# adfriend45/HYBRID9

Measured on AMD Instinct MI355X. Metric: grid-cell-steps/sec at 0.5° global (1/2/4/8 GPUs) + achieved HBM GB/s, higher is better.
Workload: dtype f32

## Files before the change

### hybrid9_amd/csrc/h9g_pair.h

```cpp
#pragma once
#include "h9g_step.h"
#if !defined(__HIPCC__) && !defined(__HIP__)
#define __device__
#define __forceinline__ inline
#endif

#ifndef H9G_EXACT_HOOK
#define H9G_EXACT_HOOK(k0, ns)
#endif
#if defined(H9G_COUNT_EXACT)
__device__ unsigned long long h9g_exact_count;
__device__ unsigned h9g_exact_wave[1 << 16];
#endif
namespace h9k {

enum : int {
  PF_TS = 0, PF_HKS, PF_BSW, PF_PSI,
  PF_NINVB,
  PF_ITS,
  PF_PTE,
  PF_C3,
  PF_ROOTR,
  PF_RPSI0, PF_RPSI1,
  PF_RTS0, PF_RTS1,
  PF_SVH2O, PF_SVSMP,
  PF_N
};
enum : int {
  PS_FMAX = 0, PS_MH3, PS_TSDZ1, PS_DAY,
  PS_LAI = PS_DAY + D_N,
  PS_LAIL, PS_PM, PS_PFM, PS_PLEN, PS_RDEPTH,
  PS_DR0,
  PS_DRS = PS_DR0 + 4 * DRP_N,
  PS_SVZWT = PS_DR0 + 2 * DR_N,
  PS_SVWA, PS_SVRNF, PS_SVERR, PS_SVNS,
  PS_N
};
enum : int { SV_ZWT = 0, SV_WA, SV_RNF, SV_ERR, SV_NS };
static_assert((PS_DAY + D_NUMC) % 2 == 0 && (PS_DAY + D_RAARAC) % 2 == 0 && (PS_DAY + D_DGRAC) % 2 == 0 &&
                  (PS_DAY + D_DRR) % 2 == 0 && (PS_DAY + D_RAC) % 2 == 0 && PS_DR0 % 2 == 0,
              "pair fields must start a row");

#ifndef H9G_FE_EQ
#define H9G_FE_EQ 1
#endif
#ifndef H9G_FE_HK
#define H9G_FE_HK 1
#endif
#ifndef H9G_FE2
#define H9G_FE2 1
#endif
#ifndef H9G_SPARE_FENCE
#define H9G_SPARE_FENCE 0
#endif
#ifndef H9G_INL_LAST
#define H9G_INL_LAST 1
#endif
#ifndef H9G_EB_FAST
#define H9G_EB_FAST 1
#endif
#ifndef H9G_HK_MDIV
#define H9G_HK_MDIV 1
#endif
#ifndef H9G_INL_MDIV
#define H9G_INL_MDIV 0
#endif
#ifndef H9G_WT_DEFER
#define H9G_WT_DEFER 1
#endif
#ifndef H9G_AQ_FREE
#define H9G_AQ_FREE 0
#endif
#ifndef H9G_SPARE_L10
#define H9G_SPARE_L10 0
#endif

#ifndef H9G_P1_TASKS
#define H9G_P1_TASKS 1
#endif

template <int K>
struct FV {
  float v[K];
};

H9K_HD float sel(int h, float a, float b) { return h ? b : a; }
H9K_HD double seld(int h, double a, double b) { return h ? b : a; }

H9K_HD float pair_swap(float v) {
#if defined(__HIP_DEVICE_COMPILE__)
  const int x = __builtin_bit_cast(int, v);
  return __builtin_bit_cast(float, __builtin_amdgcn_update_dpp(x, x, 0xB1, 0xF, 0xF, false));
#else
  return v;
#endif
}

template <int E>
H9K_HD float pair_bcast(float v) {
#if defined(__HIP_DEVICE_COMPILE__)
  const int x = __builtin_bit_cast(int, v);
  return __builtin_bit_cast(float, __builtin_amdgcn_mov_dpp(x, E ? 0xF5 : 0xA0, 0xF, 0xF, true));
#else
  return v;
#endif
}

H9K_HD float lane_get(float v, int src) {
#if defined(__HIP_DEVICE_COMPILE__)
  return __builtin_bit_cast(float, __builtin_amdgcn_ds_bpermute(src << 2, __builtin_bit_cast(int, v)));
#else
  (void)src;
  return v;
#endif
}
H9K_HD int lane_geti(int v, int src) {
#if defined(__HIP_DEVICE_COMPILE__)
  return __builtin_amdgcn_ds_bpermute(src << 2, v);
#else
  (void)src;
  return v;
#endif
}

H9K_HD float lane0_get(float v) {
#if defined(__HIP_DEVICE_COMPILE__)
  return __builtin_bit_cast(float, __builtin_amdgcn_readlane(__builtin_bit_cast(int, v), 0));
#else
  return v;
#endif
}
H9K_HD int lane0_geti(int v) {
#if defined(__HIP_DEVICE_COMPILE__)
  return __builtin_amdgcn_readlane(v, 0);
#else
  return v;
#endif
}
H9K_HD uint64_t lane_mask(bool p) {
#if defined(__HIP_DEVICE_COMPILE__)
  return __builtin_amdgcn_ballot_w64(p);
#else
  return p ? 1u : 0u;
#endif
}

H9K_HD double join_d(float lo, float hi) {
  return __builtin_bit_cast(double, (uint64_t)__builtin_bit_cast(uint32_t, hi) << 32 |
                                        __builtin_bit_cast(uint32_t, lo));
}
H9K_HD float lo_d(double v) { return __builtin_bit_cast(float, (uint32_t)__builtin_bit_cast(uint64_t, v)); }
H9K_HD float hi_d(double v) {
  return __builtin_bit_cast(float, (uint32_t)(__builtin_bit_cast(uint64_t, v) >> 32));
}

template <int L>
struct FlatStore {
  static constexpr bool kRecip = true, kRts = true, kDayRecip = true, kRtsHK = true, kSpare = false;
  static constexpr int FE_EQ = 1, FE_HK = 1;
  static constexpr int N = PF_N * L + PS_N;
  float *b;
// ... 595 lines not shown
          const float d = sp.own_sc(cs, PS_DAY + D_RAC, h);
          auto rr = [&]() __attribute__((always_inline)) { return sp.own_day_rp(cs, DRP_RA, h); };
          const float LEh = mdiv(sp.own_sc(cs, PS_DAY + D_DRR, h) + ddiv(DC(D_RHOCP) * VDD0f, d, rr),
                                 desatdT + gamma * (1.0f + ddiv(r, d, rr)));
          return FV<1>{{ddiv(LEh * 1.0E3f, DC(D_RL), [&]() { return cs.day_r(DR_RL); })}};
        },
        ft, fe);
#if defined(H9G_FORCE_RERUN)
    bad |= (__builtin_bit_cast(uint32_t, theta[1]) & 15u) == 0;
#endif
    if (!__builtin_expect(any_lane(bad), 0)) {
      rsc = rscf;
      tran = ft.v[0];
      evg = fe.v[0];
      eb_fast = true;
    }
  }
  if (!eb_fast) {
  H9G_BR(BR_EBX);
  if ((DC(D_OK) != zero) && (beta > zero))
    rsc = DC(D_X) / (DC(D_LAI2) * beta * DC(D_PW28));
  else
    rsc = 1.0E6f;
  rsc = MAXF(rsc, DC(D_RSCMIN));
  FV<2> ebc, ebs;
  sp.template pick<2>(
      [&](int h) __attribute__((always_inline)) -> FV<2> {
        const float r = sel(h, rsc, rss);
        const float q = divr<CS::kDayRecip>(m, r, sp.own_sc(cs, PS_DAY + D_RAARAC, h),
                                            [&]() { return sp.own_day_rp(cs, DRP_RAARA, h); });
        const float PM = sp.own_sc(cs, PS_DAY + D_NUMC, h) / (desatdT + gamma * (one + q));
        const float R = sp.own_sc(cs, PS_DAY + D_DGRAC, h) + gamma * r;
        return FV<2>{{PM, R}};
      },
      ebc, ebs);
  const float PMc = ebc.v[0], Rc = ebc.v[1], PMs = ebs.v[0], Rs = ebs.v[1];
  FV<1> ccf, csf;
  sp.template pick<1>(
      [&](int h) __attribute__((always_inline)) -> FV<1> {
        const float Rh = sel(h, Rc, Rs), Ro = sel(h, Rs, Rc);
        return FV<1>{{one / (one + Rh * Ra / (Ro * (Rh + Ra)))}};
      },
      ccf, csf);
  const float LE = ccf.v[0] * PMc + csf.v[0] * PMs;
  const float VDD0 = DC(D_VDD) + divr<CS::kDayRecip>(m, (DC(D_A1) - DC(D_DG) * LE) * DC(D_RAA), DC(D_RHOCP),
                                                     [&]() { return cs.day_r(DR_RHOCP); });
  FV<1> ftr, fev;
  sp.template pick<1>(
      [&](int h) __attribute__((always_inline)) -> FV<1> {
        const float r = sel(h, rsc, rss);
        const float d = sp.own_sc(cs, PS_DAY + D_RAC, h);
        auto rr = [&]() __attribute__((always_inline)) { return sp.own_day_rp(cs, DRP_RA, h); };
        const float LEh = (sp.own_sc(cs, PS_DAY + D_DRR, h) + divr<CS::kDayRecip>(m, DC(D_RHOCP) * VDD0, d, rr)) /
                          (desatdT + gamma * (1.0f + divr<CS::kDayRecip>(m, r, d, rr)));
        return FV<1>{{divr<CS::kDayRecip>(m, LEh * 1.0E3f, DC(D_RL), [&]() { return cs.day_r(DR_RL); })}};
      },
      ftr, fev);
  tran = ftr.v[0];
  evg = fev.v[0];
  }
  float em1 = m.div(g.dz(1) * (theta[1] - watmin), dt, g.rdt()) - tran * ROOT(1);
  em1 = MAXF(zero, em1);
  evg = MINF(em1, evg);
  pr.flux(evg, tran);
  const float qflx_evap = evg;
  float qflx_in_soil = (one - frac_h2osfc) * (qflx_top_soil - qflx_surf);
  qflx_in_soil = qflx_in_soil - (one - frac_h2osfc) * qflx_evap;
  const float qinmax = (one - fsat) * cs.sc(PS_MH3);
  const float qflx_infl_excess = MAXF(zero, qflx_in_soil - (one - frac_h2osfc) * qinmax);
  const float qflx_infl = qflx_in_soil - qflx_infl_excess;
  qflx_surf = qflx_surf + qflx_infl_excess;
  float zwtmm = 1000.0f * s.zwt;
  const int jwt = jwt_of<L>(s.zwt, zim);
  const bool aq = (jwt == L);
  cs.launder();
  pr.mark(1);

  float zq[L + 2];
  float hk[L + 1], dhkdw[L + 1], dsmpdw[L + 1];
  constexpr bool kTask = pair1_tasks<M, SP, CS>();
  FV<1> p0{{zero}}, p1{{zero}};
  FV<2> eA{{zero, zero}}, eS{{zero, zero}};
  bool picks = true, aq_task = false;
  {
    float *const outq[1] = {zq};
    float *const outk[4] = {hk, dhkdw, smp, dsmpdw};
    auto eq_exact = [&](int t, int h) __attribute__((always_inline)) -> FV<1> {
          H9G_BR(BR_EQX);
          const int i0 = 2 * t + 1;
          const int il = i0 + h;
          const float zlo = cs.zi(il - 1), zhi = cs.zi(il);
          const float ts = OWN(PF_TS), psi = OWN(PF_PSI);
          float vol_eq;
          if (zwtmm <= zlo) {
            vol_eq = ts;
          } else {
            const float expo = one + OWN(PF_NINVB);
            auto rp = [&]() __attribute__((always_inline)) {
              return join_d(OWN(PF_RPSI0), OWN(PF_RPSI1));
            };
            const bool inl = (zwtmm < zhi) && (zwtmm > zlo);
            const float n0 = ((-psi) + zwtmm - zlo), ni = (-psi + zwtmm - zhi);
            bool bq = false;
            float b0 = divr_d<CS::kRecip>(m, n0, -psi, rp, bq);
            float bi = divr_d<CS::kRecip>(m, ni, -psi, rp, bq);
            if (__builtin_expect(bq, 0)) {
              divr_fix<CS::kRecip>(m, b0, n0, -psi);
              divr_fix<CS::kRecip>(m, bi, ni, -psi);
            }
            bi = inl ? one : bi;
            bool s0, si;
            float temp0 = m.powf_d(b0, expo, s0);
            float tpi = m.powf_d(bi, expo, si);
            if (__builtin_expect(s0 | si, 0)) {
              m.powf_fix(temp0, b0, expo, s0);
              m.powf_fix(tpi, bi, expo, si);
            }
            if (inl) {
              const float tempi = one;
              const float voleq1 = OWN(PF_PTE) / (zwtmm - zlo) * (tempi - temp0);
              vol_eq = m.div(voleq1 * (zwtmm - zlo) + ts * (zhi - zwtmm), zhi - zlo, cs.rdz_t(il));
              vol_eq = MINF(ts, vol_eq);
              vol_eq = MAXF(vol_eq, zero);
            } else {
              const float tempi = tpi;
              vol_eq = OWN(PF_C3) * (tempi - temp0);
              vol_eq = MAXF(vol_eq, 0.0f);
              vol_eq = MINF(ts, vol_eq);
            }
          }
          const float qv = divr<CS::kRts>(m, vol_eq, ts, [&]() { return join_d(OWN(PF_RTS0), OWN(PF_RTS1)); });
          float z = psi * m.powf(MAXX(qv, 0.01f), -OWN(PF_BSW));
          return FV<1>{{MAXC(smpmin, z)}};
    };
    auto eq_body = [&](int il, auto O, float zw, bool &bad, bool inl_all) __attribute__((always_inline)) -> FV<1> {
          const float zlo = cs.zi(il - 1), zhi = cs.zi(il);
          const float ts = O(PF_TS), psi = O(PF_PSI);
          const bool sat = zw <= zlo;
          const bool inl = (zw < zhi) && (zw > zlo);
          const float expo = one + O(PF_NINVB);
          auto rp = [&]() __attribute__((always_inline)) { return join_d(O(PF_RPSI0), O(PF_RPSI1)); };
          const float n0 = ((-psi) + zw - zlo), ni = (-psi + zw - zhi);
          float b0 = divr_d<CS::kRecip>(m, n0, -psi, rp, bad);
          float bi = divr_d<CS::kRecip>(m, ni, -psi, rp, bad);
          b0 = sat ? one : b0;
          bi = (sat || inl) ? one : bi;
          bool s0, si;
          const float temp0 = m.powf_d(b0, expo, s0);
          const float tpi = m.powf_d(bi, expo, si);
          bad |= s0 | si;
          float vin = zero;
          if (inl_all || any_lane(inl)) {
          H9G_BR(BR_INL);
          const float d0 = zw - zlo;
#if H9G_INL_MDIV
          bool bq = false;
          const float q1 = mk_div(O(PF_PTE), d0, bq);
#else
          const float q1 = m.div_d(O(PF_PTE), d0, recip64(d0));
          const bool bq = m.div_bad(q1);
#endif
          const float voleq1 = q1 * (one - temp0);
          vin = m.div_d(voleq1 * (zw - zlo) + ts * (zhi - zw), zhi - zlo, cs.rdz_t(il));
          bad |= inl && (bq | m.div_bad(vin));
          vin = MINF(ts, vin);
          vin = MAXF(vin, zero);
// ... 7 lines not shown
          const float z = psi * m.powf_d(MAXX(qv, 0.01f), -O(PF_BSW), sz);
          bad |= sz;
          return FV<1>{{MAXC(smpmin, z)}};
    };
    auto eq_fast = [&](int t, int h, bool &bad) __attribute__((always_inline)) -> FV<1> {
          return eq_body(2 * t + 1 + h, [&](int p) __attribute__((always_inline)) { return OWN(p); }, zwtmm, bad,
                         false);
    };
    auto hk_exact = [&](int t, int h) __attribute__((always_inline)) -> FV<4> {
          H9G_BR(BR_HKX);
          const int i0 = 2 * t + 1;
          const int ip1 = (L < i0 + 2) ? L : i0 + 2;
          const float th = sel(h, theta[i0], theta[i0 + 1]);
          const float thp = sel(h, theta[i0 + 1], theta[ip1]);
          const float ts = OWN(PF_TS);
          const float tsp = sel(h, TS(i0 + 1), TS(ip1));
          float s1 = 0.5f * (th + thp) / (0.5f * (ts + tsp));
          s1 = MINC(one, s1);
          const float bsw = OWN(PF_BSW);
          float s_node = MAXX(divr<CS::kRtsHK>(m, th, ts, [&]() { return join_d(OWN(PF_RTS0), OWN(PF_RTS1)); }),
                              0.01f);
          s_node = MINC(one, s_node);
          const float ek = 2.0f * bsw + 2.0f, es = -bsw;
          bool sk, ss;
          float pk = m.powf_d(s1, ek, sk);
          float ps = m.powf_d(s_node, es, ss);
          if (__builtin_expect(sk | ss, 0)) {
            m.powf_fix(pk, s1, ek, sk);
            m.powf_fix(ps, s_node, es, ss);
          }
          const float s2 = OWN(PF_HKS) * pk;
          FV<4> r;
          r.v[0] = s1 * s2;
          r.v[1] = (2.0f * bsw + 3.0f) * s2 * OWN(PF_ITS);
          float sm = OWN(PF_PSI) * ps;
          sm = MAXC(smpmin, sm);
          r.v[2] = sm;
          r.v[3] = (-bsw) * sm / (s_node * ts);
          return r;
    };
    auto hk_body = [&](auto O, float th, float thp, float tsp, bool &bad) __attribute__((always_inline)) -> FV<4> {
          const float ts = O(PF_TS);
          const float sa = th + thp, sb = ts + tsp, its = O(PF_ITS);
          const float q0 = sa * its;
          float s1 = __builtin_fmaf(__builtin_fmaf(-sb, q0, sa), its, q0);
          const uint32_t ua = __builtin_bit_cast(uint32_t, sa) - 0x21800000u;
          const uint32_t ub = __builtin_bit_cast(uint32_t, sb) - 0x21800000u;
          bad |= (ua > ub ? ua : ub) >= 0x5d800000u - 0x21800000u;
          s1 = MINC(one, s1);
          const float bsw = O(PF_BSW);
          float s_node = MAXX(divr_d<CS::kRtsHK>(m, th, ts, [&]() { return join_d(O(PF_RTS0), O(PF_RTS1)); }, bad),
                              0.01f);
          s_node = MINC(one, s_node);
          const float ek = 2.0f * bsw + 2.0f, es = -bsw;
          bool sk, ss;
          const float pk = m.powf_d(s1, ek, sk);
          const float ps = m.powf_d(s_node, es, ss);
          bad |= sk | ss;
          const float s2 = O(PF_HKS) * pk;
          FV<4> r;
          r.v[0] = s1 * s2;
          r.v[1] = (2.0f * bsw + 3.0f) * s2 * O(PF_ITS);
          float sm = O(PF_PSI) * ps;
          sm = MAXC(smpmin, sm);
          r.v[2] = sm;
          if constexpr (H9G_HK_MDIV && L <= 8)
            r.v[3] = mk_div((-bsw) * sm, s_node * ts, bad);
          else
            r.v[3] = (-bsw) * sm / (s_node * ts);
          return r;
    };
    auto hk_fast = [&](int t, int h, bool &bad) __attribute__((always_inline)) -> FV<4> {
          const int i0 = 2 * t + 1;
          const int ip1 = (L < i0 + 2) ? L : i0 + 2;
          return hk_body([&](int p) __attribute__((always_inline)) { return OWN(p); }, sel(h, theta[i0], theta[i0 + 1]),
                         sel(h, theta[i0 + 1], theta[ip1]), sel(h, TS(i0 + 1), TS(ip1)), bad);
    };
    if constexpr (kTask) {
      constexpr int NA = 4 * L + 2;
      (void)outq;
      static_assert(NA <= 64 && CS::kRecip && CS::kRts && CS::kRtsHK, "a lane per task, every reciprocal stored");
      const bool st = sp.spare;
      const int hh = sp.h;
      int ln = sp.ln;
      opaque(ln);
      if (!st) {
#pragma unroll
        for (int t = 0; t < NT; t++) cs.wb[CS::TH0 + 2 * t + hh] = sel(hh, theta[2 * t + 1], theta[2 * t + 2]);
      }
      const float zw = lane0_get(zwtmm);
      const int jwu = lane0_geti(jwt);
      const bool aqu = jwu == L;
      const int jcu = aqu ? L : jwu + 1;
      const int ta = ln < NA ? ln : NA - 1;
      const bool lay_a = ta < 4 * L;
      const int ka = lay_a ? (ta & 3) : ta - 4 * L + 4;
      const int ia = lay_a ? (ta >> 2) + 1 : jcu;
      const int ipa = ia < L ? ia + 1 : L;
      const lds_float *oa = cs.wb + (ia - 1);
      const float th = oa[CS::TH0], thp = cs.wb[CS::TH0 + ipa - 1];
      const float ts_a = oa[PF_TS * L], psi_a = oa[PF_PSI * L], bsw_a = oa[PF_BSW * L];
      const float ninv_a = oa[PF_NINVB * L], its_a = oa[PF_ITS * L], hks_a = oa[PF_HKS * L];
      const float pte_a = oa[PF_PTE * L], c3_a = oa[PF_C3 * L];
      const float tsp_a = cs.wb[PF_TS * L + ipa - 1];
      const double rpsi_a = join_d(oa[PF_RPSI0 * L], oa[PF_RPSI1 * L]);
      const double rts_a = join_d(oa[PF_RTS0 * L], oa[PF_RTS1 * L]);
      const float zlo_a = cs.zi(ia - 1), zhi_a = cs.zi(ia);
      const bool sat_a = zw <= zlo_a, inl_a = (zw < zhi_a) && (zw > zlo_a);
      const float sa = th + thp, sb = ts_a + tsp_a;
      const float q0 = sa * its_a;
      float s1 = __builtin_fmaf(__builtin_fmaf(-sb, q0, sa), its_a, q0);
      const uint32_t ua = __builtin_bit_cast(uint32_t, sa) - 0x21800000u;
      const uint32_t ub = __builtin_bit_cast(uint32_t, sb) - 0x21800000u;
      const bool s1bad = (ua > ub ? ua : ub) >= 0x5d800000u - 0x21800000u;
      s1 = MINC(one, s1);
      const bool by_ts = ka == 2 || ka == 3 || (ka == 4 && !aqu);
      const float nz = (-psi_a + zw) - (ka == 0 ? zlo_a : zhi_a);
      const float num_a = by_ts ? th : (ka == 5 ? zw : nz);
      const float q_a = m.div_d(num_a, by_ts ? ts_a : -psi_a, by_ts ? rts_a : rpsi_a);
      float sn_a = MAXX(q_a, 0.01f);
      sn_a = MINC(one, sn_a);
      const bool one_a = (ka == 0 && sat_a) || (ka == 1 && (sat_a || inl_a));
      const float x_a = ka == 2 ? s1 : (by_ts ? sn_a : (ka == 5 ? one + q_a : (one_a ? one : q_a)));
      const float e_a = (ka <= 1 || (ka == 4 && aqu)) ? one + ninv_a
                        : ka == 2                     ? 2.0f * bsw_a + 2.0f
                        : ka == 3                     ? -bsw_a
                        : ka == 4                     ? 2.0f * bsw_a + 3.0f
                                                      : ninv_a;
      bool sw_a;
      const float w_a = m.powf_d(x_a, e_a, sw_a);
      bool f_a = m.div_bad(q_a) | sw_a | (ka == 2 && s1bad);
      const float s2 = hks_a * w_a;
      const float o_hk = x_a * s2;
      const float o_dhk = (2.0f * bsw_a + 3.0f) * s2 * its_a;
      float o_sm = psi_a * w_a;
      o_sm = MAXC(smpmin, o_sm);
      float o_ds;
      if constexpr (H9G_HK_MDIV && L <= 8) {
        bool b3 = false;
        o_ds = mk_div((-bsw_a) * o_sm, x_a * ts_a, b3);
        f_a |= ka == 3 && b3;
      } else {
        o_ds = (-bsw_a) * o_sm / (x_a * ts_a);
      }
      const float t0 = pair_bcast<0>(w_a);
      const bool inl1 = inl_a && ka == 1;
      float vin = zero;
      if (any_lane(inl1)) {
        H9G_BR(BR_INL);
        const float d0 = zw - zlo_a;
#if H9G_INL_MDIV
        bool bq = false;
        const float q1 = mk_div(pte_a, d0, bq);
#else
        const float q1 = m.div_d(pte_a, d0, recip64(d0));
        const bool bq = m.div_bad(q1);
#endif
        const float voleq1 = q1 * (one - t0);
        vin = m.div_d(voleq1 * (zw - zlo_a) + ts_a * (zhi_a - zw), zhi_a - zlo_a, cs.rdz_t(ia));
        f_a |= inl1 && (bq | m.div_bad(vin));
        vin = MINF(ts_a, vin);
        vin = MAXF(vin, zero);
      }
      float vbl = c3_a * (w_a - t0);
      vbl = MAXF(vbl, 0.0f);
      vbl = MINF(ts_a, vbl);
      const float vol_eq = sat_a ? ts_a : (inl_a ? vin : vbl);
      float ve = zero;
      if (aqu) {
        const float d0 = zw - g.zi(L);
        ve = pte_a / d0 * (1.0f - w_a);
        ve = MAXF(ve, 0.0f);
        ve = MINF(ts_a, ve);
      }
      const uint64_t fl_a = lane_mask(f_a);
      pr.mark(2);
      const float num_b = ka == 4 ? ve : (ka == 5 ? th : vol_eq);
      const float q_b = m.div_d(num_b, ts_a, rts_a);
      const float xm_b = MAXX(q_b, 0.01f);
      float sn_b = MAXX(0.5f * (one + q_b), 0.01f);
      sn_b = MINC(one, sn_b);
      const float x_b = ka >= 4 ? (aqu ? (ka == 4 ? xm_b : sn_b) : one) : xm_b;
      bool sw_b;
      const float w_b = m.powf_d(x_b, -bsw_a, sw_b);
      float o_z = psi_a * w_b;
      o_z = MAXC(smpmin, o_z);
      float o_dz = zero;
      if (aqu) o_dz = -bsw_a * o_z / (x_b * ts_a);
      const uint64_t fl_b = lane_mask((m.div_bad(q_b) | sw_b) && (ka == 1 || (ka >= 4 && aqu)));
      int vz = 0;
      opaque(vz);
#pragma unroll
      for (int i = 1; i <= L; i++) {
        const int lb = 4 * (i - 1);
        zq[i] = lane_get(o_z, vz + lb + 1);
        hk[i] = lane_get(o_hk, vz + lb + 2);
        dhkdw[i] = lane_get(o_dhk, vz + lb + 2);
        smp[i] = lane_get(o_sm, vz + lb + 3);
        dsmpdw[i] = lane_get(o_ds, vz + lb + 3);
      }
      p0.v[0] = lane_get(w_a, vz + 4 * L);
      p1.v[0] = lane_get(w_a, vz + 4 * L + 1);
      if (aqu) {
        eA.v[0] = lane_get(o_z, vz + 4 * L);
        eS.v[0] = lane_get(o_z, vz + 4 * L + 1);
        eS.v[1] = lane_get(o_dz, vz + 4 * L + 1);
      }
      if (st) return 0;
      constexpr uint64_t ALL_A = (1ull << (4 * L)) - 1;
      const bool bad_eq = (((fl_a & 0x3333333333333333ull) | (fl_b & 0x2222222222222222ull)) & ALL_A) != 0;
      const bool bad_hk = (fl_a & 0xCCCCCCCCCCCCCCCCull & ALL_A) != 0;
      if (__builtin_expect(bad_eq, 0)) {
#pragma unroll
        for (int t = 0; t < NT; t++) {
          const FV<1> r = eq_exact(t, hh);
          sp.xchg(r.v[0], zq[2 * t + 1], zq[2 * t + 2]);
        }
      }
      if (__builtin_expect(bad_hk, 0)) {
#pragma unroll
        for (int t = 0; t < NT; t++) {
          const FV<4> r = hk_exact(t, hh);
#pragma unroll
          for (int kk = 0; kk < 4; kk++) sp.xchg(r.v[kk], outk[kk][2 * t + 1], outk[kk][2 * t + 2]);
        }
      }
      aq_task = aqu;
      picks = ((fl_a >> (4 * L)) & 3) != 0 || (aqu && ((fl_b >> (4 * L)) & 3) != 0);
    } else if constexpr (SP::kSpare && CS::kSpare && !M::kExact) {
      constexpr int S = CS::LANES, H = 64 - S;
      constexpr int R = (NT * S + 63) / 64, U = NT - R, TOT = U * S;
      static_assert(U >= 1 && TOT <= R * H, "the helpers cover the first U slots in R rounds");
      const bool st = sp.spare;
      const int hh = sp.h;
      auto tau_q = [&](int q) __attribute__((always_inline)) {
        const int t = q * H + (st ? sp.ln - S : 0);
        return t < TOT ? t : TOT - 1;
      };
      auto src_u = [&](int u) __attribute__((always_inline)) { return S + (u * S + sp.ln) % H; };
      auto qo_u = [&](int u) __attribute__((always_inline)) { return (u * S + sp.ln) / H; };
      auto qlo = [](int u) constexpr { return (u * S) / H; };
      auto qhi = [](int u) constexpr { return ((u * S + S - 1) / H) < R - 1 ? (u * S + S - 1) / H : R - 1; };
      auto ulo = [](int q) constexpr { return (q * H) / S < U - 1 ? (q * H) / S : U - 1; };
      auto uhi = [](int q) constexpr { return (q * H + H - 1) / S < U - 1 ? (q * H + H - 1) / S : U - 1; };
      auto back = [&](const float (&v)[R], int u) __attribute__((always_inline)) {
        const int src = src_u(u), qo = qo_u(u);
        float x = lane_get(v[qlo(u)], src);
#pragma unroll
        for (int q = qlo(u) + 1; q <= qhi(u); q++) {
          const float g = lane_get(v[q], src);
          x = qo == q ? g : x;
        }
        return x;
      };
      auto flags_back = [&](int fl) __attribute__((always_inline)) {
        bool any = false;
#pragma unroll
        for (int u = 0; u < U; u++) any |= ((lane_geti(fl, src_u(u)) >> qo_u(u)) & 1) != 0;
        return any;
      };
      {
        float zwk[R];
#pragma unroll
        for (int q = 0; q < R; q++) zwk[q] = lane_get(zwtmm, tau_q(q) % S);
        FV<1> r[NT];
        float rv[R];
        int fl = 0;
#pragma unroll
        for (int q = 0; q < R; q++) {
          const int tau = tau_q(q), k = tau % S, u = tau / S;
          const int t = U + q;
          const lds_float *o = st ? cs.wb + k + u * S : cs.self + t * S;
          bool b = false;
          r[t] = eq_body(st ? 2 * u + 1 + (k & 1) : 2 * t + 1 + hh,
                         [&](int p) __attribute__((always_inline)) { return o[p * NT * S]; },
                         st ? zwk[q] : zwtmm, b, H9G_INL_LAST && U + q == NT - 1);
          rv[q] = r[t].v[0];
          fl |= (b ? 1 : 0) << q;
          if ((H9G_SPARE_FENCE >> q) & 1) sched_fence();
        }
#pragma unroll
        for (int u = 0; u < U; u++) r[u].v[0] = back(rv, u);
        const bool bad = !st & ((fl != 0) | flags_back(fl));
        if (__builtin_expect(bad, 0)) {
#pragma unroll
          for (int t = 0; t < NT; t++) r[t] = eq_exact(t, hh);
        }
#pragma unroll
        for (int t = 0; t < NT; t++) sp.xchg(r[t].v[0], zq[2 * t + 1], zq[2 * t + 2]);
      }
      pr.mark(2);
      {
        float thu[U], thpu[U];
#pragma unroll
        for (int u = 0; u < U; u++) {
          thu[u] = sel(hh, theta[2 * u + 1], theta[2 * u + 2]);
          thpu[u] = sel(hh, theta[2 * u + 2], theta[2 * u + 3]);
        }
        float thk[R], thpk[R];
#pragma unroll
        for (int q = 0; q < R; q++) {
          const int tau = tau_q(q), k = tau % S, u = tau / S;
          float a = lane_get(thu[ulo(q)], k), b = lane_get(thpu[ulo(q)], k);
#pragma unroll
          for (int w = ulo(q) + 1; w <= uhi(q); w++) {
            const float ga = lane_get(thu[w], k), gb = lane_get(thpu[w], k);
            a = u == w ? ga : a;
            b = u == w ? gb : b;
          }
          thk[q] = a;
          thpk[q] = b;
// ... 78 lines not shown
        return FV<1>{{w}};
      },
      p0, p1);
  const FV<1> pA = p0;
  if (any_aq) {
  H9G_BR(BR_ANYAQ);
  {
    const float d0 = aq ? (zwtmm - g.zi(L)) : one;
    float ve = LAYF(PF_PTE, L) / d0 * (1.0f - pA.v[0]);
    ve = MAXF(ve, 0.0f);
    ve = MINF(TS(L), ve);
    sp.template pick<2>(
        [&](int h) __attribute__((always_inline)) -> FV<2> {
          const float xn = sel(h, ve, theta[L]);
          auto xof = [&](float q2) __attribute__((always_inline)) {
            float sn = MAXX(0.5f * (one + q2), 0.01f);
            sn = MINC(one, sn);
            const float x = sel(h, MAXX(q2, 0.01f), sn);
            return aq ? x : one;
          };
          bool sq = false, sw = false;
          float q2 = divr_d<CS::kRts>(m, xn, TS(L), [&]() { return lay_d(cs, PF_RTS0, L); }, sq);
          float x = xof(q2);
          float pw = m.powf_d(x, -BSW(L), sw);
          if (__builtin_expect(sq | sw, 0)) {
            H9G_BR(BR_AQS);
            divr_fix<CS::kRts>(m, q2, xn, TS(L));
            x = xof(q2);
            pw = m.powf(x, -BSW(L));
          }
          float z = PSI(L) * pw;
          z = MAXC(smpmin, z);
          return FV<2>{{z, -BSW(L) * z / (x * TS(L))}};
        },
        eA, eS);
  }
  }
  }
  const FV<1> pY = p1;
  zq[L + 1] = aq ? eA.v[0] : zero;
  const float smp1 = eS.v[0], dsmpdw1 = eS.v[1];
  cs.launder();
  pr.mark(3);
  const float zcA = 0.5f * (zwtmm + g.zc(L));
  const float dzA = (jwt < L) ? g.dz(L) : zwtmm - g.zc(L);
  cs.launder();
  float dwat2[L + 2], GAM[L + 2];
  float BET = zero;
  double rbet = 0.0;
  int zero_pivot = 0;
  auto row = [&](int i, float am, float bm, float cm, float rm) __attribute__((always_inline)) {
    float x;
    if (i == 1) {
      BET = bm;
      x = rm;
    } else {
      BET = bm - am * GAM[i];
      if (BET == 0.0f && !zero_pivot) zero_pivot = i;
      x = rm - am * dwat2[i - 1];
    }
    rbet = recip64(BET);
    dwat2[i] = m.div_d(x, BET, rbet);
    bool bad = m.div_bad(dwat2[i]);
    if (i <= L) {
      GAM[i + 1] = m.div_d(cm, BET, rbet);
      bad |= m.div_bad(GAM[i + 1]);
    }
    if (__builtin_expect(bad, 0)) {
      m.div_fix(dwat2[i], x, BET);
      if (i <= L) m.div_fix(GAM[i + 1], cm, BET);
    }
  };
  bool tri_ok = false;
  if constexpr (!M::kExact) {
    bool bad = false, zp = false;
    float qo[L + 1], d1[L + 1], d2[L + 1];
    auto flux3_f = [&](float hki, float num, float dsi, float dsn, float dhk, float den, double rden, int k,
                       bool &b) __attribute__((always_inline)) {
      qo[k] = m.div_d(-hki * num, den, rden);
      d1[k] = m.div_d(-(-hki * dsi + num * dhk), den, rden);
      d2[k] = m.div_d(-(hki * dsn + num * dhk), den, rden);
      b |= m.div_bad(qo[k]) | m.div_bad(d1[k]) | m.div_bad(d2[k]);
    };
#pragma unroll
    for (int i = 1; i <= L - 1; i++)
      flux3_f(hk[i], (smp[i + 1] - smp[i]) - (zq[i + 1] - zq[i]), dsmpdw[i], dsmpdw[i + 1], dhkdw[i], g.den(i),
              g.rden(i), i, bad);
    qo[L] = d1[L] = d2[L] = zero;
    if (any_aq) {
      const float den = zcA - g.zc(L);
      bool ba = false;
      flux3_f(hk[L], smp1 - smp[L] - (zq[L + 1] - zq[L]), dsmpdw[L], dsmpdw1, dhkdw[L], den, recip64(den), L, ba);
      bad |= aq && ba;
    }
    if (__builtin_expect(bad, 0)) {
      H9G_BR(BR_TRIFLUX);
#pragma unroll
      for (int i = 1; i <= L; i++) {
        const bool a = i == L;
        const float num = a ? smp1 - smp[L] - (zq[L + 1] - zq[L]) : (smp[i + 1] - smp[i]) - (zq[i + 1] - zq[i]);
        const float dsn = a ? dsmpdw1 : dsmpdw[i < L ? i + 1 : L];
        const float den = a ? zcA - g.zc(L) : g.den(i);
        m.div_fix(qo[i], -hk[i] * num, den);
        m.div_fix(d1[i], -(-hk[i] * dsmpdw[i] + num * dhkdw[i]), den);
        m.div_fix(d2[i], -(hk[i] * dsn + num * dhkdw[i]), den);
      }
      bad = false;
    }
    auto row_f = [&](int i, float am, float bm, float cm, float rm) __attribute__((always_inline)) {
      float x;
      if (i == 1) {
        BET = bm;
        x = rm;
      } else {
        BET = bm - am * GAM[i];
        zp |= BET == 0.0f;
        x = rm - am * dwat2[i - 1];
      }
      const double rb = recip64(BET);
      dwat2[i] = m.div_d(x, BET, rb);
      bad |= m.div_bad(dwat2[i]);
      if (i <= L) {
        GAM[i + 1] = m.div_d(cm, BET, rb);
        bad |= m.div_bad(GAM[i + 1]);
      }
    };
    auto dzdt = [&](float dz) __attribute__((always_inline)) {
      const float q = m.div_d(dz, dt, g.rdt());
      bad |= m.div_bad(q);
      return q;
    };
    const float bm1 = dzdt(g.dz(1)) + d1[1];
    row_f(1, zero, bm1, d2[1], qflx_infl - qo[1] - tran * ROOT(1));
#pragma unroll
    for (int i = 2; i <= L - 1; i++)
      row_f(i, -d1[i - 1], dzdt(g.dz(i)) - d2[i - 1] + d1[i], d2[i], qo[i - 1] - qo[i] - tran * ROOT(i));
    row_f(L, -d1[L - 1], dzdt(g.dz(L)) - d2[L - 1] + (aq ? d1[L] : zero), aq ? d2[L] : zero,
          qo[L - 1] - (aq ? qo[L] : zero) - tran * ROOT(L));
    const float qA = dzdt(dzA);
    const float bmA = qA - d2[L] + zero;
    const float rmA = qo[L] - zero;
    row_f(L + 1, aq ? -d1[L] : zero, aq ? bmA : qA, zero, aq ? rmA : zero);
    if (__builtin_expect(bad | zp | (bm1 == 0.0f), 0)) {
      H9G_BR(BR_TRISWEEP);
      BET = zero;
      zero_pivot = 0;
      const float bm1x = m.div(g.dz(1), dt, g.rdt()) + d1[1];
      if (bm1x == 0.0f) { errval = bm1x; return 1; }
      row(1, zero, bm1x, d2[1], qflx_infl - qo[1] - tran * ROOT(1));
#pragma unroll
      for (int i = 2; i <= L - 1; i++)
        row(i, -d1[i - 1], m.div(g.dz(i), dt, g.rdt()) - d2[i - 1] + d1[i], d2[i], qo[i - 1] - qo[i] - tran * ROOT(i));
      if (!aq) {
        row(L, -d1[L - 1], m.div(g.dz(L), dt, g.rdt()) - d2[L - 1] + zero, zero, qo[L - 1] - zero - tran * ROOT(L));
        row(L + 1, zero, m.div(dzA, dt, g.rdt()), zero, zero);
      } else {
        row(L, -d1[L - 1], m.div(g.dz(L), dt, g.rdt()) - d2[L - 1] + d1[L], d2[L], qo[L - 1] - qo[L] - tran * ROOT(L));
        row(L + 1, -d1[L], m.div(dzA, dt, g.rdt()) - d2[L] + zero, zero, qo[L] - zero);
      }
      if (zero_pivot) { errval = (float)zero_pivot; return 2; }
    }
    tri_ok = true;
  }
  if (!tri_ok) {
  auto flux3 = [&](float hki, float num, float dsi, float dsn, float dhk, float den, double rden, float &qo,
                   float &d1, float &d2) __attribute__((always_inline)) {
    const float x0 = -hki * num, x1 = -(-hki * dsi + num * dhk), x2 = -(hki * dsn + num * dhk);
    qo = m.div_d(x0, den, rden);
    d1 = m.div_d(x1, den, rden);
    d2 = m.div_d(x2, den, rden);
    if (__builtin_expect(m.div_bad(qo) | m.div_bad(d1) | m.div_bad(d2), 0)) {
      m.div_fix(qo, x0, den);
      m.div_fix(d1, x1, den);
      m.div_fix(d2, x2, den);
    }
  };
  float q_prev, dq0_prev, dq1_prev;
  {
    const float den = g.den(1);
    const double rden = g.rden(1);
    const float dzq = (zq[2] - zq[1]);
    const float num = (smp[2] - smp[1]) - dzq;
    float qout, dqodw1, dqodw2;
    flux3(hk[1], num, dsmpdw[1], dsmpdw[2], dhkdw[1], den, rden, qout, dqodw1, dqodw2);
    const float bm1 = m.div(g.dz(1), dt, g.rdt()) + dqodw1;
    if (bm1 == 0.0f) { errval = bm1; return 1; }
    row(1, zero, bm1, dqodw2, qflx_infl - qout - tran * ROOT(1));
    q_prev = qout; dq0_prev = dqodw1; dq1_prev = dqodw2;
  }
#pragma unroll
  for (int i = 2; i <= L - 1; i++) {
    const float den = g.den(i);
    const double rden = g.rden(i);
    const float dzq = zq[i + 1] - zq[i];
    const float num = (smp[i + 1] - smp[i]) - dzq;
    float qout, dqodw1, dqodw2;
    flux3(hk[i], num, dsmpdw[i], dsmpdw[i + 1], dhkdw[i], den, rden, qout, dqodw1, dqodw2);
    row(i, -dq0_prev, m.div(g.dz(i), dt, g.rdt()) - dq1_prev + dqodw1, dqodw2,
        q_prev - qout - tran * ROOT(i));
    q_prev = qout; dq0_prev = dqodw1; dq1_prev = dqodw2;
  }
  {
    constexpr int i = L;
    if (i > jwt) {
      const float qout = zero, dqodw1 = zero;
      row(i, -dq0_prev, m.div(g.dz(i), dt, g.rdt()) - dq1_prev + dqodw1, zero,
          q_prev - qout - tran * ROOT(i));
      row(i + 1, zero, m.div(dzA, dt, g.rdt()), zero, zero);
    } else {
      const float den = zcA - g.zc(i);
      const double rden = recip64(den);
      const float dzq = zq[i + 1] - zq[i];
      const float num = smp1 - smp[i] - dzq;
      float qout, dqodw1, dqodw2;
      flux3(hk[i], num, dsmpdw[i], dsmpdw1, dhkdw[i], den, rden, qout, dqodw1, dqodw2);
      row(i, -dq0_prev, m.div(g.dz(i), dt, g.rdt()) - dq1_prev + dqodw1, dqodw2,
          q_prev - qout - tran * ROOT(i));
      const float qout1 = zero, dqodw1b = zero;
      row(i + 1, -dqodw1, m.div(dzA, dt, g.rdt()) - dqodw2 + dqodw1b, zero, qout - qout1);
    }
  }
  if (zero_pivot) { errval = (float)zero_pivot; return 2; }
  }
#pragma unroll
  for (int i = L; i >= 1; i--) dwat2[i] = dwat2[i] - GAM[i + 1] * dwat2[i + 1];
#pragma unroll
  for (int i = 1; i <= L; i++) h2o[i] = h2o[i] + dwat2[i] * g.dz(i);
  cs.launder();
  pr.mark(4);
  auto s_y_base = [&](int i, float zmm) __attribute__((always_inline)) -> float {
    return one + divr<CS::kRecip>(m, zmm, -cs.lay(PF_PSI, i), [&]() { return lay_d(cs, PF_RPSI0, i); });
  };
  auto s_y_of = [&](int i, float pw) __attribute__((always_inline)) -> float {
    return MAXX(cs.lay(PF_TS, i) * (one - pw), 0.02f);
  };
  auto s_y_at = [&](int i, float zmm) __attribute__((always_inline)) -> float {
    return s_y_of(i, m.powf(s_y_base(i, zmm), cs.lay(PF_NINVB, i)));
  };
  float qcharge, sy_first = zero;
  if (jwt < L) {
    H9G_BR(BR_JWTCOL);
    const int j1 = jwt + 1;
    const float hks_j = cs.lay(PF_HKS, j1);
    float smp_m = zero, zq_m = zero, zc_j = zero;
#pragma unroll
    for (int i = 1; i <= L; i++) {
      if (i == (jwt > 1 ? jwt : 1)) { smp_m = smp[i]; zq_m = zq[i]; }
      if (i == jwt) zc_j = g.zc(i);
    }
    const float wh_zwt = zero;
    sy_first = s_y_of(jwt + 1, p1.v[0]);
    const float ka = hks_j * p0.v[0];
    const float smp1m = MAXC(smpmin, smp_m);
    const float wh = smp1m - zq_m;
    if (jwt == 0)
      qcharge = -ka * (wh_zwt - wh) / (zwtmm + one);
    else
      qcharge = -ka * (wh_zwt - wh) / ((zwtmm - zc_j) * 2.0f);
    qcharge = MAXC(-10.0f / dt, qcharge);
    qcharge = MINC(10.0f / dt, qcharge);
  } else {
    qcharge = m.div(dwat2[L + 1] * dzA, dt, g.rdt());
  }
  float rous = MAXX(TS(L) * (one - pY.v[0]), 0.02f);
  auto wdiv = [&](float x) __attribute__((always_inline)) {
    if constexpr (H9G_WT_DEFER && !M::kExact) {
      const float q = m.div_d(x, 1000.0f, r1000);
      m.special |= m.div_bad(q);
      return q;
    } else {
      return m.div(x, 1000.0f, r1000);
    }
  };
  int jwt2 = jwt;
  if (jwt == L) {
    s.wa = s.wa + qcharge * dt;
    s.zwt = s.zwt - m.div(qcharge * dt, 1000.0f, r1000) / rous;
  } else {
    float qcharge_tot = qcharge * dt;
    if (qcharge_tot > zero) {
      visit_layers(m, [&](int k) __attribute__((always_inline)) -> bool {
        const int i = jwt + 1 - k;
        const float s_y = k == 0 ? sy_first : s_y_at(i, zwtmm);
        float qcl = MINF(qcharge_tot, s_y * (zwtmm - cs.zi(i - 1)));
        qcl = MAXF(qcl, zero);
        if (s_y > zero) s.zwt = s.zwt - wdiv(qcl / s_y);
        qcharge_tot = qcharge_tot - qcl;
        return !(qcharge_tot <= zero || i == 1);
      });
    } else {
      visit_layers(m, [&](int k) __attribute__((always_inline)) -> bool {
        const int i = jwt + 1 + k;
        const float s_y = k == 0 ? sy_first : s_y_at(i, zwtmm);
        float qcl = MAXF(qcharge_tot, -s_y * (cs.zi(i) - zwtmm));
        qcl = MINF(qcl, zero);
        qcharge_tot = qcharge_tot - qcl;
        if (qcharge_tot >= zero) {
          s.zwt = s.zwt - wdiv(qcl / s_y);
          return false;
        }
        s.zwt = cs.zim(i);
        return i != L;
      });
      if (qcharge_tot > zero) {
        if (!aq) rous = s_y_at(L, zwtmm);
        s.zwt = s.zwt - wdiv(qcharge_tot) / rous;
      }
    }
    jwt2 = jwt_of<L>(s.zwt, zim);
  }
  cs.launder();
  pr.mark(5);
  zwtmm = 1000.0f * s.zwt;
  float rsub_top;
  const int jd = jwt2 < L ? jwt2 + 1 : L;
  FV<1> pR, pD;
  sp.template pick<1>(
      [&](int h) __attribute__((always_inline)) -> FV<1> {
        const int i = h ? jd : L;
        bool se = false, sq = false, sw = false;
        float ex = expf_fast(m, -fff * s.zwt, se);
        const float nb = -cs.lay(PF_PSI, i);
        float q = divr_d<CS::kRecip>(m, zwtmm, nb, [&]() { return lay_d(cs, PF_RPSI0, i); }, sq);
        float w = m.powf_d(one + q, cs.lay(PF_NINVB, i), sw);
        if (__builtin_expect(se | sq | sw, 0)) {
          H9G_BR(BR_BASE);
          if (se) ex = m.expf(-fff * s.zwt);
          divr_fix<CS::kRecip>(m, q, zwtmm, nb);
          w = m.powf(one + q, cs.lay(PF_NINVB, i));
        }
        rsub_top = 5.5E-3f * ex;
// ... 429 lines not shown
```

### hybrid9_amd/csrc/h9g_step.h

```cpp
#pragma once
#include "h9_math.h"
#include "h9g_geo.h"

namespace h9k {

constexpr float zero = 0.0f, one = 1.0f;
constexpr int H9G_ERR_NOSNAP_K = 5;
constexpr float rhow = 1000.0f;
constexpr float gasc = 8.314510f;
constexpr float rgas = 0x1.1f0c7cp+8f;
constexpr float deltx = 0x1.3738bcp-1f;
constexpr float stbo = 5.67E-8f;
constexpr float tf = 273.16f;
constexpr float smpmin = -1.0E8f;
constexpr float cp = 1010.0f;
constexpr float watmin = 0.01f;
constexpr float sla1 = 23.0E-3f;
constexpr float log_0p1 = -0x1.26bb1cp+1f;

#if defined(H9G_FASTMINMAX) && defined(__HIP_DEVICE_COMPILE__)
H9K_HD float MAXF(float a, float b) { return __builtin_fmaxf(a, b); }
H9K_HD float MINF(float a, float b) { return __builtin_fminf(a, b); }
#else
H9K_HD float MAXF(float a, float b) { return a > b ? a : b; }
// ... 14 lines not shown
  return MINF(c, x);
#endif
}
H9K_HD float MAXX(float x, float c) {
#if defined(__HIP_DEVICE_COMPILE__)
  return __builtin_fmaxf(x, c);
#else
  return MAXF(x, c);
#endif
}

#ifndef H9G_FENCE_MASK
#define H9G_FENCE_MASK 0x100
#endif
H9K_HD void sched_fence() {
#if defined(__HIP_DEVICE_COMPILE__) && !defined(H9G_NOFENCE)
  __builtin_amdgcn_sched_barrier(H9G_FENCE_MASK);
#endif
}

template <class T>
H9K_HD void opaque(T &x) {
#if defined(__HIP_DEVICE_COMPILE__)
  asm volatile("" : "+v"(x));
#else
  (void)x;
#endif
}

H9K_HD bool any_lane(bool p) {
#if defined(__HIP_DEVICE_COMPILE__)
  return __builtin_amdgcn_ballot_w64(p) != 0;
#else
  return p;
#endif
}

#if defined(H9G_COUNT_BRANCH)
__device__ unsigned long long h9g_branch_count[64];
#endif
#if defined(H9G_COUNT_BRANCH) && defined(__HIP_DEVICE_COMPILE__)
#define H9G_BR(k)                                                                   \
  do {                                                                              \
    const uint64_t em_ = __builtin_amdgcn_read_exec();                              \
    if (__lane_id() == (unsigned)__builtin_ctzll(em_)) {                            \
      atomicAdd(&h9g_branch_count[(k)], 1ull);                                      \
      atomicAdd(&h9g_branch_count[32 + (k)], (unsigned long long)__builtin_popcountll(em_)); \
    }                                                                               \
  } while (0)
#else
#define H9G_BR(k) ((void)0)
#endif
#if defined(H9G_DUMP_AQ)
__device__ unsigned *h9g_aq_bits;
__device__ const float *h9g_aq_base;
#endif
enum : int {
  BR_SUBSTEP = 0, BR_THETA, BR_QB, BR_EQX, BR_AQPOW, BR_AQS, BR_HKX, BR_TRIFLUX, BR_TRISWEEP, BR_RECH,
  BR_BASE, BR_WATMIN, BR_RERUN, BR_POWREDO, BR_DIVREDO, BR_EXPREDO, BR_POWFIX, BR_DIVFIX, BR_INL, BR_ANYAQ,
  BR_JWTCOL, BR_VISIT2, BR_SNAP, BR_EBX, BR_DAY, BR_N
};

H9K_HD bool bad_quotient(float q) {
#if defined(__HIP_DEVICE_COMPILE__)
  return __builtin_amdgcn_classf(q, 0x093);
#else
  const uint32_t u = __builtin_bit_cast(uint32_t, q) & 0x7fffffffu;
  return (u != 0 && u < 0x00800000u) || u > 0x7f800000u;
#endif
}

H9K_HD float mk_div(float x, float d, bool &bad) {
#if defined(__HIP_DEVICE_COMPILE__)
  const float r = __builtin_amdgcn_rcpf(d);
#else
  const float r = 1.0f / d;
#endif
  const float y = __builtin_fmaf(__builtin_fmaf(-d, r, 1.0f), r, r);
  const float q0 = x * y;
  const float q = __builtin_fmaf(__builtin_fmaf(-d, q0, x), y, q0);
  const uint32_t ux = (__builtin_bit_cast(uint32_t, x) & 0x7fffffffu) - 0x21800000u;
  const uint32_t ud = (__builtin_bit_cast(uint32_t, d) & 0x7fffffffu) - 0x21800000u;
  bad |= (ux > ud ? ux : ud) >= 0x5d800000u - 0x21800000u;
  return q;
}

H9K_HD double recip64(float d) {
  const double dd = (double)d;
#if defined(__HIP_DEVICE_COMPILE__)
  double r = __builtin_amdgcn_rcp(dd);
#else
  double r = 1.0 / dd;
#endif
  double e = __builtin_fma(-dd, r, 1.0);
  r = __builtin_fma(r, e, r);
  e = __builtin_fma(-dd, r, 1.0);
  r = __builtin_fma(r, e, r);
  return r;
}

struct MathExact {
  static constexpr bool kExact = true;
  h9m::Tabs T;
  H9K_HD float expf(float x) { return h9m::expf(x, T); }
  H9K_HD float powf(float x, float y) { return h9m::powf(x, y, T); }
  H9K_HD float div(float x, float d, double) { return x / d; }
  H9K_HD float powf_d(float x, float y, bool &sp) {
    sp = false;
    return h9m::powf(x, y, T);
  }
  H9K_HD void powf_fix(float &, float, float, bool) {}
  H9K_HD float div_d(float x, float d, double) { return x / d; }
  H9K_HD bool div_bad(float) const { return false; }
  H9K_HD void div_fix(float &, float, float) {}
};
#if defined(__HIP_DEVICE_COMPILE__) && defined(H9G_RARE_CALLS)
#define H9K_RARE __device__ __attribute__((noinline, cold))
#elif defined(__HIP_DEVICE_COMPILE__)
#define H9K_RARE __device__ __forceinline__
#else
#define H9K_RARE static __attribute__((noinline, cold))
#endif

H9K_RARE float expf_redo(float x, const uint64_t *e2, const double *l2) { return h9m::expf(x, {e2, l2}); }
H9K_RARE float powf_redo(float x, float y, const uint64_t *e2, const double *l2) {
  return h9m::powf(x, y, {e2, l2});
}

struct MathFast {
  static constexpr bool kExact = false;
  h9m::Tabs T;
  bool special;
  unsigned redone = 0;
  H9K_HD float expf(float x) {
    bool sp = false;
    float r = h9m::expf_nx(x, T, sp);
    if (__builtin_expect(sp, 0)) {
      H9G_BR(BR_EXPREDO);
      r = expf_redo(x, T.exp2, T.log2);
      redone++;
    }
    return r;
  }
  H9K_HD float powf(float x, float y) {
    bool sp = false;
    float r = h9m::powf_nx<false>(x, y, T, sp);
    if (__builtin_expect(sp, 0)) {
      H9G_BR(BR_POWREDO);
      r = powf_redo(x, y, T.exp2, T.log2);
      redone++;
    }
    return r;
  }
  H9K_HD float div(float x, float d, double r) {
    float q = (float)((double)x * r);
    if (__builtin_expect(bad_quotient(q), 0)) {
      H9G_BR(BR_DIVREDO);
      q = x / d;
      redone++;
    }
    return q;
  }
  H9K_HD float powf_d(float x, float y, bool &sp) {
    sp = false;
    return h9m::powf_nx<false>(x, y, T, sp);
  }
// ... 238 lines not shown
```

Before: 4.134 billion.

## Compute soil flux coefficients lane-parallel in task path and use fast divides

Enables new task-mode bits that compute the per-interface flux coefficients (qout, dqodw1, dqodw2) one lane per layer inside the wavefront task layout. Only those coefficients and smp are broadcast back, and the full per-layer gathers plus the serial flux loop run only on a slow path when any flag is bad. It also caches the recharge smp/zq lookup, and swaps the float64-reciprocal divides in the tridiagonal rows for float32 mk_div with range checks. This cuts serial flux arithmetic and lane broadcasts, at the cost of more register arrays, extra branching, and a new fallback-correctness path.

```diff
diff --git a/hybrid9_amd/csrc/h9g_pair.h b/hybrid9_amd/csrc/h9g_pair.h
--- a/hybrid9_amd/csrc/h9g_pair.h
+++ b/hybrid9_amd/csrc/h9g_pair.h
@@ -76,7 +76,7 @@
 #endif
 
 #ifndef H9G_P1_TASKS
-#define H9G_P1_TASKS 1
+#define H9G_P1_TASKS 7
 #endif
 
 template <int K>
@@ -838,6 +838,9 @@
   FV<1> p0{{zero}}, p1{{zero}};
   FV<2> eA{{zero, zero}}, eS{{zero, zero}};
   bool picks = true, aq_task = false;
+  float c_q[L + 1], c_1[L + 1], c_2[L + 1];
+  bool flux_done = false;
+  float rc_smp = zero, rc_zq = zero;
   {
     float *const outq[1] = {zq};
     float *const outk[4] = {hk, dhkdw, smp, dsmpdw};
@@ -1011,6 +1014,17 @@
       static_assert(NA <= 64 && CS::kRecip && CS::kRts && CS::kRtsHK, "a lane per task, every reciprocal stored");
       const bool st = sp.spare;
       const int hh = sp.h;
+#if (H9G_P1_TASKS & 2)
+      float den_l = g.den(1);
+      double rden_l = g.rden(1);
+#pragma unroll
+      for (int i = 2; i <= L - 1; i++)
+        if ((sp.ln >> 2) + 1 == i) {
+          den_l = g.den(i);
+          rden_l = g.rden(i);
+        }
+      float c_qo, c_d1, c_d2;
+#endif
       int ln = sp.ln;
       opaque(ln);
       if (!st) {
@@ -1117,28 +1131,82 @@
       float o_dz = zero;
       if (aqu) o_dz = -bsw_a * o_z / (x_b * ts_a);
       const uint64_t fl_b = lane_mask((m.div_bad(q_b) | sw_b) && (ka == 1 || (ka >= 4 && aqu)));
-      int vz = 0;
-      opaque(vz);
-#pragma unroll
-      for (int i = 1; i <= L; i++) {
-        const int lb = 4 * (i - 1);
-        zq[i] = lane_get(o_z, vz + lb + 1);
-        hk[i] = lane_get(o_hk, vz + lb + 2);
-        dhkdw[i] = lane_get(o_dhk, vz + lb + 2);
-        smp[i] = lane_get(o_sm, vz + lb + 3);
-        dsmpdw[i] = lane_get(o_ds, vz + lb + 3);
-      }
-      p0.v[0] = lane_get(w_a, vz + 4 * L);
-      p1.v[0] = lane_get(w_a, vz + 4 * L + 1);
-      if (aqu) {
-        eA.v[0] = lane_get(o_z, vz + 4 * L);
-        eS.v[0] = lane_get(o_z, vz + 4 * L + 1);
-        eS.v[1] = lane_get(o_dz, vz + 4 * L + 1);
-      }
-      if (st) return 0;
       constexpr uint64_t ALL_A = (1ull << (4 * L)) - 1;
       const bool bad_eq = (((fl_a & 0x3333333333333333ull) | (fl_b & 0x2222222222222222ull)) & ALL_A) != 0;
       const bool bad_hk = (fl_a & 0xCCCCCCCCCCCCCCCCull & ALL_A) != 0;
+      const bool bad_pk = ((fl_a >> (4 * L)) & 3) != 0 || (aqu && ((fl_b >> (4 * L)) & 3) != 0);
+      int vz = 0;
+      opaque(vz);
+      bool slow = true;
+#if (H9G_P1_TASKS & 2)
+      {
+        const bool top = ia == L;
+        const float n_sm = ka == 5 ? o_z : o_sm, n_ds = ka == 5 ? o_dz : o_ds;
+        const int sn = top ? 4 * L + 1 : ln + 5, zn = top ? 4 * L : ln + 3;
+        const float sm_i = lane_get(o_sm, (ln + 1) & 63), ds_i = lane_get(o_ds, (ln + 1) & 63);
+        const float sm_n = lane_get(n_sm, sn & 63), ds_n = lane_get(n_ds, sn & 63);
+        const float zq_i = lane_get(o_z, (ln + 63) & 63), zq_n = lane_get(o_z, zn & 63);
+        float den_c = den_l;
+        double rden_c = rden_l;
+        if (aqu) {
+          const float zcA_c = 0.5f * (zw + g.zc(L));
+          const float dA = zcA_c - g.zc(L);
+          const double rA = recip64(dA);
+          den_c = top ? dA : den_c;
+          rden_c = top ? rA : rden_c;
+        }
+        const float num = (sm_n - sm_i) - (zq_n - zq_i);
+        c_qo = m.div_d(-o_hk * num, den_c, rden_c);
+        c_d1 = m.div_d(-(-o_hk * ds_i + num * o_dhk), den_c, rden_c);
+        c_d2 = m.div_d(-(o_hk * ds_n + num * o_dhk), den_c, rden_c);
+        bool f_c = (m.div_bad(c_qo) | m.div_bad(c_d1) | m.div_bad(c_d2)) && ka == 2 && (!top || aqu);
+#if defined(H9G_FORCE_RERUN)
+        f_c |= (__builtin_bit_cast(uint32_t, zw) & 1u) == 0;
+#endif
+        slow = bad_eq | bad_hk | bad_pk | (lane_mask(f_c) != 0);
+      }
+#pragma unroll
+      for (int i = 1; i <= L; i++) {
+        const int lb = 4 * (i - 1);
+        smp[i] = lane_get(o_sm, vz + lb + 3);
+        if (i < L) {
+          c_q[i] = lane_get(c_qo, vz + lb + 2);
+          c_1[i] = lane_get(c_d1, vz + lb + 2);
+          c_2[i] = lane_get(c_d2, vz + lb + 2);
+        }
+      }
+      c_q[L] = c_1[L] = c_2[L] = zero;
+      if (aqu) {
+        c_q[L] = lane_get(c_qo, vz + 4 * L - 2);
+        c_1[L] = lane_get(c_d1, vz + 4 * L - 2);
+        c_2[L] = lane_get(c_d2, vz + 4 * L - 2);
+      }
+      {
+        const int lm = 4 * ((jwu > 1 ? jwu : 1) - 1);
+        rc_smp = lane_get(o_sm, vz + lm + 3);
+        rc_zq = lane_get(o_z, vz + lm + 1);
+      }
+#endif
+      p0.v[0] = lane_get(w_a, vz + 4 * L);
+      p1.v[0] = lane_get(w_a, vz + 4 * L + 1);
+      if (__builtin_expect(slow, 0)) {
+#pragma unroll
+        for (int i = 1; i <= L; i++) {
+          const int lb = 4 * (i - 1);
+          zq[i] = lane_get(o_z, vz + lb + 1);
+          hk[i] = lane_get(o_hk, vz + lb + 2);
+          dhkdw[i] = lane_get(o_dhk, vz + lb + 2);
+          smp[i] = lane_get(o_sm, vz + lb + 3);
+          dsmpdw[i] = lane_get(o_ds, vz + lb + 3);
+        }
+        if (aqu) {
+          eA.v[0] = lane_get(o_z, vz + 4 * L);
+          eS.v[0] = lane_get(o_z, vz + 4 * L + 1);
+          eS.v[1] = lane_get(o_dz, vz + 4 * L + 1);
+        }
+      }
+      if (st) return 0;
+      flux_done = !slow;
       if (__builtin_expect(bad_eq, 0)) {
 #pragma unroll
         for (int t = 0; t < NT; t++) {
@@ -1154,8 +1222,15 @@
           for (int kk = 0; kk < 4; kk++) sp.xchg(r.v[kk], outk[kk][2 * t + 1], outk[kk][2 * t + 2]);
         }
       }
+#if (H9G_P1_TASKS & 2)
+      if (__builtin_expect(slow, 0)) {
+#pragma unroll
+        for (int i = 1; i <= L; i++)
+          if (i == (jwt > 1 ? jwt : 1)) { rc_smp = smp[i]; rc_zq = zq[i]; }
+      }
+#endif
       aq_task = aqu;
-      picks = ((fl_a >> (4 * L)) & 3) != 0 || (aqu && ((fl_b >> (4 * L)) & 3) != 0);
+      picks = bad_pk;
     } else if constexpr (SP::kSpare && CS::kSpare && !M::kExact) {
       constexpr int S = CS::LANES, H = 64 - S;
       constexpr int R = (NT * S + 63) / 64, U = NT - R, TOT = U * S;
@@ -1400,6 +1475,15 @@
       d2[k] = m.div_d(-(hki * dsn + num * dhk), den, rden);
       b |= m.div_bad(qo[k]) | m.div_bad(d1[k]) | m.div_bad(d2[k]);
     };
+    if constexpr (kTask && (H9G_P1_TASKS & 2)) {
+#pragma unroll
+      for (int i = 1; i <= L; i++) {
+        qo[i] = c_q[i];
+        d1[i] = c_1[i];
+        d2[i] = c_2[i];
+      }
+    }
+    if (!kTask || __builtin_expect(!flux_done, 0)) {
 #pragma unroll
     for (int i = 1; i <= L - 1; i++)
       flux3_f(hk[i], (smp[i + 1] - smp[i]) - (zq[i + 1] - zq[i]), dsmpdw[i], dsmpdw[i + 1], dhkdw[i], g.den(i),
@@ -1425,6 +1509,7 @@
       }
       bad = false;
     }
+    }
     auto row_f = [&](int i, float am, float bm, float cm, float rm) __attribute__((always_inline)) {
       float x;
       if (i == 1) {
@@ -1435,12 +1520,17 @@
         zp |= BET == 0.0f;
         x = rm - am * dwat2[i - 1];
       }
+      if constexpr (kTask && (H9G_P1_TASKS & 4)) {
+        dwat2[i] = i == L + 1 ? mk_div_z(x, BET, bad) : mk_div(x, BET, bad);
+        if (i <= L) GAM[i + 1] = i == L ? mk_div_z(cm, BET, bad) : mk_div(cm, BET, bad);
+      } else {
       const double rb = recip64(BET);
       dwat2[i] = m.div_d(x, BET, rb);
       bad |= m.div_bad(dwat2[i]);
       if (i <= L) {
         GAM[i + 1] = m.div_d(cm, BET, rb);
         bad |= m.div_bad(GAM[i + 1]);
+      }
       }
     };
     auto dzdt = [&](float dz) __attribute__((always_inline)) {
@@ -1561,10 +1651,18 @@
     const int j1 = jwt + 1;
     const float hks_j = cs.lay(PF_HKS, j1);
     float smp_m = zero, zq_m = zero, zc_j = zero;
+    if constexpr (kTask && (H9G_P1_TASKS & 2)) {
+      smp_m = rc_smp;
+      zq_m = rc_zq;
+#pragma unroll
+      for (int i = 1; i <= L; i++)
+        if (i == jwt) zc_j = g.zc(i);
+    } else {
 #pragma unroll
     for (int i = 1; i <= L; i++) {
       if (i == (jwt > 1 ? jwt : 1)) { smp_m = smp[i]; zq_m = zq[i]; }
       if (i == jwt) zc_j = g.zc(i);
+    }
     }
     const float wh_zwt = zero;
     sy_first = s_y_of(jwt + 1, p1.v[0]);
diff --git a/hybrid9_amd/csrc/h9g_step.h b/hybrid9_amd/csrc/h9g_step.h
--- a/hybrid9_amd/csrc/h9g_step.h
+++ b/hybrid9_amd/csrc/h9g_step.h
@@ -120,6 +120,13 @@
   const uint32_t ux = (__builtin_bit_cast(uint32_t, x) & 0x7fffffffu) - 0x21800000u;
   const uint32_t ud = (__builtin_bit_cast(uint32_t, d) & 0x7fffffffu) - 0x21800000u;
   bad |= (ux > ud ? ux : ud) >= 0x5d800000u - 0x21800000u;
+  return q;
+}
+H9K_HD float mk_div_z(float x, float d, bool &bad) {
+  bool b = false;
+  const float q = mk_div(x, d, b);
+  const uint32_t ud = (__builtin_bit_cast(uint32_t, d) & 0x7fffffffu) - 0x21800000u;
+  bad |= __builtin_bit_cast(uint32_t, x) == 0u ? ud >= 0x5d800000u - 0x21800000u : b;
   return q;
 }
 
```

After: 4.306 billion (median of 6 runs). +4.2%, better.
